# zbqq/neus2

Hardware: AMD Instinct MI355X
Metric: training samples/sec (compacted NeuS2 training samples, DTU-scan24-shaped synthetic, base.json) (higher is better)
Workload: dtype fp16 MFMA (fp32 accumulate) / fp32 optimizer; 1 GPU; NeuS2 train step, Config S, base.json L=14 T=2^19 W=64, Nc=2^18/GPU, R=2^18/GPU fixed, all 14 levels active (network trained 800 steps before the warm-up); global_batch=262144, rays_per_gpu=262144, parallelism=dp1, prepare_steps=800, levels_active=14

## Files before the change

include/neus2_hip.h:

```cpp
#ifndef NEUS2_HIP_H
#define NEUS2_HIP_H

#include <stdint.h>

#ifdef __cplusplus
extern "C" {
#endif

typedef struct NeusTestbed NeusTestbed;

typedef struct NeusNetworkConfig {
	uint32_t n_levels;
	uint32_t n_features_per_level;
	uint32_t log2_hashmap_size;
	uint32_t base_resolution;
	float per_level_scale;
	float top_resolution;
	float valid_level_scale;
	float base_valid_level_scale;
	uint32_t base_training_step;
	uint32_t n_neurons;
	uint32_t n_density_hidden;
	uint32_t n_rgb_hidden;
	float learning_rate, beta1, beta2, epsilon, l2_reg;
// ... 154 lines not shown
int neus_testbed_ray_counts(NeusTestbed* tb, uint32_t n, uint32_t* nreq, uint32_t* ccount, uint32_t* numsteps );
int neus_debug_time_kernel(NeusTestbed* tb, int kernel, int variant, int iters, float* ms_out);
int neus_testbed_time_kernel(NeusTestbed* tb, int kernel, int iters, float* ms_out, uint32_t* units_out);
int neus_debug_march_stats(NeusTestbed* tb, uint32_t n, uint32_t* out);
int neus_debug_march_profile(NeusTestbed* tb, unsigned long long* out, uint32_t max_waves, uint32_t* n_waves);
int neus_debug_scatter_stats(NeusTestbed* tb, uint64_t* records_per_level, uint32_t* max_region);
int neus_debug_scatter_parts(NeusTestbed* tb, uint32_t* parts_per_level );
int neus_debug_grid_scatter(NeusTestbed* tb, void* hip_stream, uint32_t n_cap, const uint32_t* n_valid, const float* coords,
                            uint32_t coord_stride, uint32_t valid_level, const void* dLdenc, const void* genc, const float* v,
                            float* grid_grad_out);
int neus_debug_mlp_train(NeusTestbed* tb, void* hip_stream, uint32_t n, const float* coords, const uint16_t* enc, const float* dydx,
                         const uint16_t* dL_dout, uint32_t indeed_batch_size, float* grads_out, float* dpos, uint16_t* genc_out,
                         uint16_t* dLdenc_out, uint16_t* d1_delta_out, float* v_out);
int neus_debug_exclusive_scan(void* hip_stream, const uint32_t* in, uint32_t* out, uint32_t n, int reps, uint32_t* failures);
int neus_debug_scan_giveup(void* hip_stream, const uint32_t* in, uint32_t* out, uint32_t n, uint32_t* failures);
int neus_debug_inject_health(NeusTestbed* tb, uint32_t flags);
int neus_debug_set_lds_fill(NeusTestbed* tb, uint32_t pattern);
int neus_debug_set_lds_fill_all(NeusTestbed* tb, uint32_t pattern);
int neus_debug_set_xcd_shift(NeusTestbed* tb, uint32_t n_blocks);
int neus_debug_set_grid_generic(uint32_t on);
int neus_debug_get_batch(NeusTestbed* tb, float* coords_out, uint16_t* dl_dout_out, float* loss_out);
int neus_debug_denorm_probe(int device, uint32_t n, uint32_t launches, uint64_t* stats);
int neus_debug_get_buffer(NeusTestbed* tb, int id, uint64_t offset, uint64_t nbytes, void* host);
int neus_debug_replay_loss_grad(NeusTestbed* tb, uint16_t* dl_dout_out);
int neus_debug_sample_rays_round0(NeusTestbed* tb, void* stream, uint32_t n_rays, uint32_t n_rays_total, uint64_t rng_state, uint64_t rng_inc,
                                  uint32_t max_samples, const uint8_t* bitfield, float* rays, uint32_t* numsteps, float* coords,
                                  uint32_t* counters_out, uint32_t chunk_end, uint32_t* list, uint32_t* list_len, uint32_t lds_fill);
int neus_testbed_stream(NeusTestbed* tb, void** hip_stream);
int neus_testbed_synchronize(NeusTestbed* tb);
#define NEUS_N_PHASES 10
// ... 110 lines not shown
```

neus2_amd/_lib.py:

```python
from __future__ import annotations

import ctypes as C
import os

_HERE = os.path.dirname(os.path.abspath(__file__))
LIB_PATH = os.environ.get("NEUS2_HIP_LIB") or os.path.join(_HERE, "libneus2_hip.so")


class NeusNetworkConfig(C.Structure):
    _fields_ = [
        ("n_levels", C.c_uint32), ("n_features_per_level", C.c_uint32), ("log2_hashmap_size", C.c_uint32),
        ("base_resolution", C.c_uint32), ("per_level_scale", C.c_float), ("top_resolution", C.c_float),
        ("valid_level_scale", C.c_float), ("base_valid_level_scale", C.c_float), ("base_training_step", C.c_uint32),
        ("n_neurons", C.c_uint32), ("n_density_hidden", C.c_uint32), ("n_rgb_hidden", C.c_uint32),
        ("learning_rate", C.c_float), ("beta1", C.c_float), ("beta2", C.c_float), ("epsilon", C.c_float), ("l2_reg", C.c_float),
        ("ema_decay", C.c_float), ("decay_start", C.c_uint32), ("decay_interval", C.c_uint32), ("decay_base", C.c_float),
        ("ek_loss_weight", C.c_float), ("mask_loss_weight", C.c_float), ("anneal_end", C.c_uint32), ("batch_size", C.c_uint32),
        ("sdf_bias", C.c_float), ("density_grid_decay", C.c_float), ("seed", C.c_uint32), ("fixed_rays_per_batch", C.c_uint32),
        ("predict_global_movement", C.c_uint32), ("global_movement_steps", C.c_uint32), ("finetune_global_movement", C.c_uint32),
        ("reset_density_grid_after_global_movement", C.c_uint32), ("after_learning_rate", C.c_float),
        ("gm_learning_rate", C.c_float), ("gm_beta1", C.c_float), ("gm_beta2", C.c_float), ("gm_epsilon", C.c_float),
        ("gm_decay_start", C.c_uint32), ("gm_decay_interval", C.c_uint32), ("gm_decay_base", C.c_float),
    ]

# ... 68 lines not shown

class NeusModuleInfo(C.Structure):
    _fields_ = [("n_params", C.c_uint64), ("n_input_dims", C.c_uint32), ("n_output_dims", C.c_uint32),
                ("param_precision", C.c_int32), ("output_precision", C.c_int32), ("gradient_precision", C.c_int32),
                ("batch_capacity", C.c_uint32), ("n_levels", C.c_uint32), ("grid_offset", C.c_uint64),
                ("per_level_scale", C.c_float)]


EXPORTS = [
    "neus_last_error", "neus_abi_version", "neus_device_count", "neus_device_synchronize",
    "neus_testbed_create", "neus_testbed_destroy", "neus_testbed_set_dataset", "neus_testbed_reload_network",
    "neus_testbed_layout", "neus_testbed_train", "neus_testbed_get_stats", "neus_testbed_get_params",
    "neus_testbed_set_params", "neus_testbed_get_gradients", "neus_testbed_get_ema_params",
    "neus_testbed_get_half_params",
    "neus_testbed_get_density_grid", "neus_testbed_set_density_grid", "neus_testbed_restore_state", "neus_testbed_get_rng", "neus_testbed_render", "neus_testbed_sdf_on_grid",
    "neus_testbed_marching_cubes", "neus_testbed_mc_density", "neus_testbed_get_mesh", "neus_testbed_mesh_vertex_colors", "neus_mc_table", "neus_prepare_image_rgba8", "neus_testbed_ray_counts", "neus_debug_time_kernel", "neus_debug_march_stats", "neus_debug_exclusive_scan", "neus_debug_scan_giveup", "neus_debug_inject_health", "neus_debug_set_lds_fill", "neus_debug_set_lds_fill_all", "neus_debug_set_xcd_shift", "neus_debug_set_grid_generic", "neus_debug_denorm_probe", "neus_debug_get_batch", "neus_debug_get_buffer", "neus_debug_replay_loss_grad", "neus_debug_sample_rays_round0", "neus_debug_march_profile", "neus_debug_scatter_stats", "neus_debug_scatter_parts", "neus_debug_grid_scatter", "neus_debug_mlp_train", "neus_testbed_time_kernel", "neus_testbed_stream",
    "neus_testbed_synchronize", "neus_testbed_set_profiling", "neus_testbed_kernel_times", "neus_testbed_set_infer_timing", "neus_testbed_infer_timing",
    "neus_testbed_set_exchange_timing", "neus_testbed_exchange_timing",
    "neus_nccl_unique_id", "neus_testbed_init_data_parallel", "neus_testbed_init_data_parallel_ex",
    "neus_testbed_data_parallel_info", "neus_testbed_set_exchange_overlap", "neus_local_group_create", "neus_local_group_destroy",
    "neus_testbed_init_local_group", "neus_host_group_create", "neus_host_group_destroy", "neus_testbed_init_host_group", "neus_debug_host_group_allreduce",
    "neus_grid_encode", "neus_net_forward", "neus_net_backward", "neus_sample_rays", "neus_loss_compact",
    "neus_optimizer_step", "neus_fill_rollover", "neus_occ_update", "neus_mfma_probe",
    "neus_testbed_next_frame", "neus_testbed_get_movement", "neus_testbed_set_movement", "neus_testbed_frame_state",
    "neus_testbed_change_frame", "neus_testbed_prepare_for_test", "neus_testbed_get_training_options",
    "neus_testbed_set_training_options", "neus_testbed_saved_transform", "neus_testbed_get_optimizer_state",
    "neus_testbed_set_optimizer_state", "neus_testbed_set_progressive_inference",
    "neus_module_create_network", "neus_module_create_nerf_network", "neus_module_create_encoding", "neus_module_create_network_with_input_encoding", "neus_module_destroy", "neus_context_destroy",
    "neus_module_info", "neus_module_hyperparams", "neus_module_set_training_step", "neus_module_set_indeed_batch_size",
    "neus_module_initialize_params", "neus_module_inference", "neus_module_forward", "neus_module_backward",
    "neus_module_backward_backward_input",
# ... 39 lines not shown
```

neus2_amd/csrc/kernels.h:

```cpp
#pragma once
#include <functional>
#include <vector>
#include "common.h"

namespace neus {

struct MlpPtrs {
	const half_t* d0;  const half_t* d1;
	const half_t* r0;  const half_t* r1;  const half_t* r2;
	const half_t* d0T; const half_t* d1T;
	const half_t* r0T; const half_t* r1T; const half_t* r2T;
	const half_t* d0p; const half_t* d0Tp;
	const half_t* var;
	float sdf_bias;
};

struct TrainBufs {
	half_t* d1_delta;
	half_t* dLdenc; half_t* genc;
	float4* v;
	float* var_grad;
	float* var_partial;
	float indeed_batch;
	float4* dpos;
// ... 87 lines not shown

struct LossWork {
	float4* sa;
	float4* ck4;
	float* cke;
	float* ekt;
	uint32_t* sample_ray;
	const uint32_t* rbase;
	float4* racc;
	float* rT;
	float* rek;
	uint32_t* long_rays;
	uint32_t* n_long;
	float4* rgr;
	uint32_t* cmap;
};

constexpr uint32_t ADAM_BIAS_TAB = 4096;
struct AdamParams {
	uint32_t n, n_matrix;
	float loss_scale, lr, beta1, beta2, eps, l2_reg;
	float ema_decay, ema_debias_old, ema_debias_new;
	uint32_t optimize_matrix, optimize_non_matrix;
	const float* bias_tab;
	uint32_t bias_converged;
	float inv_loss_scale;
	uint32_t pow2_scale;
	uint32_t skip_ema_h;
	const uint32_t* abort;
};
// ... 278 lines not shown
```

neus2_amd/csrc/march.hip:

```cpp
#pragma clang fp contract(off)
#include "march_common.h"
#include "scan_lookback.h"
#include <algorithm>
#include <cstdlib>
#include <cstring>
#include <vector>

namespace neus {



__global__ void k_bitfield_linear(const uint8_t* __restrict__ bf, uint32_t* __restrict__ lin) {
	const uint32_t w = blockIdx.x * blockDim.x + threadIdx.x;
	if (w >= GRID3 / 32) return;
	const uint32_t ix = w >> 9, iy = (w >> 2) & 127, iz0 = (w & 3) * 32;
	uint32_t word = 0;
	for (uint32_t b = 0; b < 32; ++b) {
		const uint32_t idx = morton3D(ix, iy, iz0 + b);
		word |= (uint32_t)((bf[idx / 8] >> (idx % 8)) & 1) << b;
	}
	lin[w] = word;
}
__device__ __forceinline__ bool ray_hits_box(const float o[3], const float d[3], const float bb[6]) {
	float tn = 0.0f, tf = 3.402823466e+38f;
// ... 1143 lines not shown
						for (uint32_t j = lane; j < m_o; j += 64) list[p_o + j] = s_o + j;
					}
				}
				if (rays_out) {
					const unsigned long long mk = __ballot(m > 0);
					uint32_t q0 = 0;
					if (lane == 0) q0 = atomicAdd(n_rays_out, (uint32_t)__popcll(mk));
					q0 = wave_lane_value(q0, 0);
					if (m > 0) rays_out[q0 + (uint32_t)__popcll(mk & ((1ull << lane) - 1ull))] = i;
				}
			}
		}
	}
}

__global__ void __launch_bounds__(256) k_prog_cut(uint32_t cap_rays, const uint32_t* __restrict__ ccount, const uint32_t* __restrict__ excl,
                                                  uint32_t batch, uint32_t* __restrict__ cutw, int mode, uint32_t* __restrict__ eval0,
                                                  uint32_t* __restrict__ abort_if_none) {
	const uint32_t i = blockIdx.x * blockDim.x + threadIdx.x;
	if (i >= cap_rays) return;
	const uint32_t e = excl[i], incl = e + ccount[i];
	const bool cross = e < batch && incl >= batch, none = i == cap_rays - 1 && incl < batch;
	if (!cross && !none) return;
	const uint32_t c = cross ? i : cap_rays;
	if (mode == 0) {
		cutw[CW_CUT_A] = c;
		cutw[CW_LENB_EFF] = cross ? 0u : cutw[CW_LENB];
		cutw[CW_NB_EFF] = cross ? 0u : cutw[CW_NB];
	} else {
		cutw[CW_CUT] = c;
// ... 92 lines not shown
                                                  float4* __restrict__ racc, const float* __restrict__ rT, float4* __restrict__ rgr,
                                                  float* __restrict__ loss_out, float* __restrict__ ek_out, float* __restrict__ mask_out,
                                                  uint32_t* __restrict__ cmap) {
	const uint32_t lane = threadIdx.x & 63;
	const uint32_t R = st->rays_per_batch;
	const uint32_t n_rays_global = R * dp.world, n_rays_total = st->n_rays_total;
	const uint32_t cap64 = (cap_rays + 63u) & ~63u;
	const uint32_t mi_lb = st->mi_lb;
	if (lp.abort_w && blockIdx.x == 0 && threadIdx.x == 0) lp.abort_w[lp.abort_slot ^ 1u] = 0u;
	for (uint32_t i = blockIdx.x * blockDim.x + threadIdx.x; i < cap64; i += gridDim.x * blockDim.x) {
		uint32_t comp = 0, cb = 0;
		if (i < cap_rays) {
			const uint32_t ns = numsteps[2 * i], base = numsteps[2 * i + 1];
			const uint32_t cn = ccount[i];
			cb = cbase[i];
			if (i == cap_rays - 1) {
				if (lp.abort_w && st->march_cut && cb + cn < lp.max_compacted) lp.abort_w[lp.abort_slot] = 1u;
				st->compacted_counter = cb + cn;
				st->compacted_global = cb + cn;
				st->rays_ws_global = st->n_rays_with_samples;
				st->n_train = min(cb + cn, lp.max_compacted) ? lp.max_compacted : 0u;
			}
			loss_out[i] = 0.f; ek_out[i] = 0.f; mask_out[i] = 0.f;
			if (ns == 0) {
				numsteps[2 * i] = 0; numsteps[2 * i + 1] = cb;
			} else {
				const float4 acc = racc[i];
				float rgb_ray[3] = {acc.x, acc.y, acc.z}, weight_sum = acc.w;
				const float T = rT[i];
				const uint32_t ig = dp.rank * R + i;
				pcg32 rng(lp.rng_state, lp.rng_inc);
				pcg_advance(rng, (uint64_t)(uint32_t)(ig * N_MAX_RANDOM_SAMPLES_PER_RAY), lp.jt);
				const uint32_t img = image_idx(ig, n_rays_global, n_rays_total, ds.n_images);
				const int rx = ds.res[2 * img], ry = ds.res[2 * img + 1];
				float xx, yy; random_image_pos(rng, rx, ry, xx, yy);
				float bg[3];
				if (ds.target.fixed_bg) { bg[0] = ds.target.bg[0]; bg[1] = ds.target.bg[1]; bg[2] = ds.target.bg[2]; }
				else { bg[0] = rng.next_float(); bg[1] = rng.next_float(); bg[2] = rng.next_float(); }
	#pragma unroll
				for (int k = 0; k < 3; ++k) bg[k] = srgb_to_linear(bg[k]);
				float tex[4]; read_rgba(ds, img, xx, yy, tex);
				float target[3];
				const uint32_t tmode = ds.target.mode;
	#pragma unroll
				for (int k = 0; k < 3; ++k) {
					if (tmode != 1) {
						target[k] = 1.0f * tex[k] + (1.0f - tex[3]) * bg[k];
						if (tmode == 0) { target[k] = linear_to_srgb(target[k]); bg[k] = linear_to_srgb(bg[k]); }
					} else {
						bg[k] = linear_to_srgb(bg[k]);
						target[k] = tex[3] > 0.0f ? linear_to_srgb(1.0f * tex[k] / tex[3]) * tex[3] + (1.0f - tex[3]) * bg[k] : bg[k];
					}
				}
				if (cn == ns) {
	#pragma unroll
					for (int k = 0; k < 3; ++k) rgb_ray[k] += T * bg[k];
				}
				comp = min(lp.max_compacted - min(lp.max_compacted, cb), cn);
				if (lp.abort_w && mi_lb && comp > 0 && base + ns > mi_lb) lp.abort_w[lp.abort_slot] = 1u;
				numsteps[2 * i] = comp; numsteps[2 * i + 1] = cb;
				if (comp > 0) {
					float lgrad[3], lloss[3];
	#pragma unroll
					for (int k = 0; k < 3; ++k) {
						const float diff = rgb_ray[k] - target[k], ad = fabsf(diff), sq = 0.5f / 0.1f * diff * diff;
						lloss[k] = (ad > 0.1f ? (ad - 0.5f * 0.1f) : sq) / 5.0f;
						lgrad[k] = (ad > 0.1f ? (diff > 0 ? 1.0f : -1.0f) : (diff / 0.1f)) / 5.0f;
					}
					const float mask_gt = (float)(tex[3] > 0.9999f);
					float gws;
					if (weight_sum >= 1.0 - 1e-4) { weight_sum = 1.0 - 1e-4; gws = 0.0f; }
					else if (weight_sum <= 1e-4) { weight_sum = 1e-4; gws = 0.0f; }
					else { const float sws = 1.0f / (1.0f + exp(-(double)weight_sum)); gws = (mask_gt - sws) * weight_sum * lp.mask_w; }
					const float mean_loss = ((lloss[0] + lloss[1]) + lloss[2]) / 3.0f;
					loss_out[i] = mean_loss / (float)n_rays_global;
					mask_out[i] = -(mask_gt * logf(weight_sum) + (1 - mask_gt) * logf(1 - weight_sum));
					float Tb;
					const RecState sc = scan_replay(base, base + comp - 1, sa, ekt, ck4, cke, Tb);
					ek_out[i] = sc.ek / ((float)comp * (float)n_rays_global);
					rgr[i] = make_float4(lgrad[0], lgrad[1], lgrad[2], gws * (1 - weight_sum));
					racc[i] = make_float4(rgb_ray[0], rgb_ray[1], rgb_ray[2], 0.f);
				}
			}
		}
		unsigned long long todo = __ballot(comp > 0);
		const uint32_t i0 = i - lane;
		while (todo) {
			const int o = __ffsll(todo) - 1;
			todo &= todo - 1ull;
			const uint32_t c_o = wave_lane_value(comp, o), d_o = wave_lane_value(cb, o);
			for (uint32_t j = lane; j < c_o; j += 64) cmap[d_o + j] = i0 + (uint32_t)o;
		}
	}
}
// ... 244 lines not shown
void launch_loss_alpha(hipStream_t s, uint32_t cap_samples, const StepState* st, const float* coords, const half_t* net_out, float cos_anneal,
                       const LossWork& w, bool dt_const) {
	dbg_lds_gate(s);
	k_loss_alpha<<<sample_blocks(cap_samples), 256, 0, s>>>(cap_samples, &st->n_kept, nullptr, coords, net_out, cos_anneal, w.sa, w.ekt, w.n_long,
	                                                        dt_const);
}
void launch_loss_alpha_list(hipStream_t s, uint32_t cap_samples, const uint32_t* n_ptr, const uint32_t* idx, const float* coords,
                            const half_t* net_out, float cos_anneal, const LossWork& w, bool dt_const) {
	dbg_lds_gate(s);
	k_loss_alpha<<<sample_blocks(cap_samples), 256, 0, s>>>(cap_samples, n_ptr, idx, coords, net_out, cos_anneal, w.sa, w.ekt, nullptr, dt_const);
}
void launch_loss_scan_chunk(hipStream_t s, uint32_t cap_rays, const uint32_t* numsteps, const LossWork& w, uint32_t* ccount, uint32_t e0,
                            uint32_t e1, uint32_t e2, uint32_t* list, uint32_t* next_counter, const uint32_t* rays_in, const uint32_t* n_rays_in,
                            uint32_t* rays_out, uint32_t* n_rays_out) {
	dbg_lds_gate(s);
	k_loss_scan_chunk<<<std::max<uint32_t>(1, std::min<uint32_t>((cap_rays + 63) / 64, 8192)), 64, 0, s>>>(
		cap_rays, numsteps, w.sa, w.ekt, w.ck4, w.cke, ccount, w.racc, w.rT, w.rek, e0, e1, e2, list, next_counter, rays_in, n_rays_in,
		rays_out, n_rays_out);
}
void launch_prog_cut(hipStream_t s, uint32_t cap_rays, const uint32_t* ccount, const uint32_t* excl, uint32_t batch, uint32_t* cutw, int mode,
                     uint32_t* eval0, uint32_t* abort_if_none) {
	k_prog_cut<<<(cap_rays + 255) / 256, 256, 0, s>>>(cap_rays, ccount, excl, batch, cutw, mode, eval0, abort_if_none);
}
void launch_prog_next(hipStream_t s, uint32_t cap_rays, const uint32_t* rays_in, const uint32_t* n_in, const uint32_t* numsteps, const uint32_t* cut,
                      uint32_t e1, uint32_t e2, uint32_t* list, uint32_t* list_counter, uint32_t* rays_out, uint32_t* n_out) {
	k_prog_next<<<std::max<uint32_t>(1, std::min<uint32_t>((cap_rays + 255) / 256, 1024)), 256, 0, s>>>(rays_in, n_in, numsteps, cut, e1, e2, list,
	                                                                                                   list_counter, rays_out, n_out);
}
void launch_loss_scan_ray(hipStream_t s, uint32_t cap_rays, const uint32_t* numsteps, const LossWork& w, uint32_t* ccount) {
	const uint32_t blocks = ray_blocks(cap_rays);
	dbg_lds_gate(s);
	k_loss_scan_ray<true><<<blocks, 256, 0, s>>>(cap_rays, numsteps, w.sa, w.ekt, w.ck4, w.cke, ccount, w.racc, w.rT, w.long_rays, w.n_long);
	if (w.long_rays) dbg_lds_gate(s);
// ... 44 lines not shown
```

neus2_amd/csrc/march_common.h:

```cpp
#pragma once
#pragma clang fp contract(off)
#include "kernels.h"

namespace neus {

__device__ __forceinline__ float clampf(float v, float lo, float hi) { return v < lo ? lo : (v > hi ? hi : v); }
__device__ __forceinline__ float calc_dt(float t, float cone) { return clampf(t * cone, MIN_CONE_STEPSIZE, MAX_CONE_STEPSIZE); }
__device__ __forceinline__ float warp_dt(float dt) {
	const float max_stepsize = MIN_CONE_STEPSIZE * (1 << (NERF_CASCADES - 1));
	return (dt - MIN_CONE_STEPSIZE) / (max_stepsize - MIN_CONE_STEPSIZE);
}
__device__ __forceinline__ float unwarp_dt(float dt) {
	const float max_stepsize = MIN_CONE_STEPSIZE * (1 << (NERF_CASCADES - 1));
	return dt * (max_stepsize - MIN_CONE_STEPSIZE) + MIN_CONE_STEPSIZE;
}
__device__ __forceinline__ int clampi(int v, int lo, int hi) { return v < lo ? lo : (v > hi ? hi : v); }
__device__ __forceinline__ uint32_t cascaded_grid_idx_at(float px, float py, float pz, uint32_t mip) {
	const float s = scalbnf(1.0f, -(int)mip);
	px = ((px - 0.5f) * s) + 0.5f; py = ((py - 0.5f) * s) + 0.5f; pz = ((pz - 0.5f) * s) + 0.5f;
	const int ix = (int)(px * NERF_GRIDSIZE), iy = (int)(py * NERF_GRIDSIZE), iz = (int)(pz * NERF_GRIDSIZE);
	return morton3D(clampi(ix, 0, NERF_GRIDSIZE - 1), clampi(iy, 0, NERF_GRIDSIZE - 1), clampi(iz, 0, NERF_GRIDSIZE - 1));
}
__device__ __forceinline__ bool occupied(float px, float py, float pz, const uint8_t* bf, uint32_t mip) {
	const uint32_t idx = cascaded_grid_idx_at(px, py, pz, mip);
// ... 41 lines not shown
	do { t += calc_dt(t, cone); } while (t < t_target);
	return t;
}
__device__ __forceinline__ float srgb_to_linear(float s) { return s <= 0.04045f ? s / 12.92f : powf((s + 0.055f) / 1.055f, 2.4f); }
__device__ __forceinline__ float linear_to_srgb(float l) { return l < 0.0031308f ? 12.92f * l : 1.055f * powf(l, 0.41666f) - 0.055f; }

__device__ __forceinline__ uint32_t image_idx(uint32_t base_idx, uint32_t n_rays, uint32_t n_rays_total, uint32_t n_img) {
	return (((base_idx + n_rays_total) * n_img) / n_rays) % n_img;
}
__device__ __forceinline__ void random_image_pos(pcg32& rng, int rx, int ry, float& x, float& y) {
	x = rng.next_float(); y = rng.next_float();
	const int ix = min(max((int)(x * (float)rx), 0), rx - 1);
	const int iy = min(max((int)(y * (float)ry), 0), ry - 1);
	x = ((float)ix + 0.5f) / (float)rx; y = ((float)iy + 0.5f) / (float)ry;
}
__device__ __forceinline__ void read_rgba(const DevDataset& ds, uint32_t img, float x, float y, float o[4]) {
	const int rx = ds.res[2 * img], ry = ds.res[2 * img + 1];
	const int px = clampi((int)(x * (float)rx), 0, rx - 1), py = clampi((int)(y * (float)ry), 0, ry - 1);
	const uint32_t v = ds.pixels[ds.pix_off[img] + (uint64_t)px + (uint64_t)py * rx];
	if (v == 0x00FF00FFu) { o[0] = o[1] = o[2] = o[3] = -1.0f; return; }
	const float a = (float)((v >> 24) & 0xff) * (1.0f / 255.0f);
	o[0] = ds.lin_lut[v & 0xff] * a;
	o[1] = ds.lin_lut[(v >> 8) & 0xff] * a;
	o[2] = ds.lin_lut[(v >> 16) & 0xff] * a;
	o[3] = a;
}
__device__ __forceinline__ bool aabb_contains(const DevDataset& ds, const float p[3]) {
	return (p[0] >= ds.aabb_min[0]) & (p[0] <= ds.aabb_max[0]) & (p[1] >= ds.aabb_min[1]) & (p[1] <= ds.aabb_max[1]) &
	       (p[2] >= ds.aabb_min[2]) & (p[2] <= ds.aabb_max[2]);
}
__device__ __forceinline__ void ray_intersect(const DevDataset& ds, const float o[3], const float d[3], float& tmin_o) {
	float tmin = (ds.aabb_min[0] - o[0]) / d[0], tmax = (ds.aabb_max[0] - o[0]) / d[0];
	if (tmin > tmax) { float t = tmin; tmin = tmax; tmax = t; }
	float tymin = (ds.aabb_min[1] - o[1]) / d[1], tymax = (ds.aabb_max[1] - o[1]) / d[1];
	if (tymin > tymax) { float t = tymin; tymin = tymax; tymax = t; }
	const float FM = 3.402823466e+38f;
	if (tmin > tymax || tymin > tmax) { tmin_o = FM; return; }
	if (tymin > tmin) tmin = tymin;
	if (tymax < tmax) tmax = tymax;
	float tzmin = (ds.aabb_min[2] - o[2]) / d[2], tzmax = (ds.aabb_max[2] - o[2]) / d[2];
// ... 99 lines not shown
```

neus2_amd/csrc/options.h:

```cpp
#pragma once

#include <algorithm>
#include <cstdint>
#include <cstdio>
#include <cstdlib>
#include <cstring>
#include <vector>

namespace neus_env {
inline bool on_unless_0(const char* name) { const char* e = std::getenv(name); return !(e && e[0] == '0'); }
inline bool off_unless_1(const char* name) { const char* e = std::getenv(name); return e && e[0] == '1'; }
inline bool is(const char* name, const char* value) { const char* e = std::getenv(name); return e && std::strcmp(e, value) == 0; }
inline int as_int(const char* name, int def) { const char* e = std::getenv(name); return e ? std::atoi(e) : def; }
inline uint32_t as_u32(const char* name, uint32_t def) { const char* e = std::getenv(name); return e ? (uint32_t)std::strtoul(e, nullptr, 10) : def; }
inline float as_float(const char* name, float def) { const char* e = std::getenv(name); return e ? (float)std::atof(e) : def; }
inline std::vector<uint32_t> increasing_list(const char* name) {
	std::vector<uint32_t> v;
	const char* e = std::getenv(name);
	if (!e) return v;
	for (const char* p = e; *p;) { char* q = nullptr; const unsigned long x = std::strtoul(p, &q, 10); if (q == p) break; v.push_back((uint32_t)x); p = *q ? q + 1 : q; }
	bool ok = !v.empty() && v.size() <= 14 && v[0] > 0;
	for (size_t k = 1; k < v.size(); ++k) ok = ok && v[k] > v[k - 1];
	if (!ok) v.clear();
	return v;
// ... 13 lines not shown
	bool eager_ema_h = false;

	uint32_t march_waves = 0;
	uint32_t march_lanes = 8;
	bool march_balance = true;
	uint32_t march_dbg = 0;
	bool ray_cull = true;
	bool ray_sort = true;
	bool prog_cut = true;
	bool march_cut = true;
	uint32_t march_cut_div = 1;
	std::vector<uint32_t> chunk_ends;
	float chunk_scale = 2.f;
	int chunk_rounds = 2;

	bool occ_sort = true;
	bool occ_nu_sort = false;

	uint32_t scatter_mode = 2;
	uint32_t scatter_chunk = 512;
	uint32_t scatter_level_groups = 0;
	uint32_t scatter_xcd_group = 4;
	bool scatter_noskip = false;

	bool dbg_loss_replay = false;
	bool dbg_loss_fence = false;

	static NeusOptions from_env() {
		using namespace neus_env;
		NeusOptions o;
// ... 7 lines not shown
		o.adam_overlap = off_unless_1("NEUS_ADAM_OVERLAP");
		o.exchange_overlap = on_unless_0("NEUS_EXCHANGE_OVERLAP");
		o.eager_ema_h = off_unless_1("NEUS_EAGER_EMA_H");
		o.march_waves = as_u32("NEUS_MARCH_WAVES", o.march_waves);
		{ const uint32_t v = as_u32("NEUS_MARCH_LANES", 8); o.march_lanes = v == 1 || v == 4 || v == 16 ? v : 8u; }
		o.march_balance = on_unless_0("NEUS_MARCH_BALANCE");
		o.march_dbg = as_u32("NEUS_MARCH_DBG", o.march_dbg);
		o.ray_cull = on_unless_0("NEUS_RAY_CULL");
		o.ray_sort = on_unless_0("NEUS_RAY_SORT");
		o.prog_cut = on_unless_0("NEUS_PROG_CUT");
		o.march_cut = on_unless_0("NEUS_MARCH_CUT");
		o.march_cut_div = (uint32_t)std::max(1, as_int("NEUS_DBG_MARCH_CUT_DIV", 1));
		o.chunk_ends = increasing_list("NEUS_CHUNK_ENDS");
		o.chunk_scale = as_float("NEUS_CHUNK_SCALE", o.chunk_scale);
		o.chunk_rounds = as_int("NEUS_CHUNK_ROUNDS", o.chunk_rounds);
		o.occ_sort = on_unless_0("NEUS_OCC_SORT");
		o.occ_nu_sort = off_unless_1("NEUS_OCC_NU_SORT");
		o.scatter_mode = is("NEUS_SCATTER", "binned") ? 1u : is("NEUS_SCATTER", "wide") ? 0u : 2u;
		o.scatter_chunk = is("NEUS_SCATTER_CHUNK", "1024") ? 1024u : is("NEUS_SCATTER_CHUNK", "256") ? 256u : 512u;
		if (o.scatter_mode != 2 && o.scatter_chunk == 256) o.scatter_chunk = 512;
		o.scatter_level_groups = (uint32_t)std::max(0, as_int("NEUS_SCATTER_LG", 0));
		o.scatter_xcd_group = std::max(1u, as_u32("NEUS_SC_XCD_GROUP", o.scatter_xcd_group));
		o.scatter_noskip = off_unless_1("NEUS_SCATTER_NOSKIP");
		o.dbg_loss_replay = off_unless_1("NEUS_DBG_LOSS_REPLAY");
		o.dbg_loss_fence = off_unless_1("NEUS_DBG_LOSS_FENCE");
		return o;
	}
};

struct NeusProcessOptions {
// ... 32 lines not shown
```

neus2_amd/csrc/testbed.cpp:

```cpp
#include <rocprofiler-sdk-roctx/roctx.h>
#include "kernels.h"
#include "scan_lookback.h"
#include "json_lite.h"
#include "hostgroup.h"
#include "options.h"
#include "../../include/neus2_hip.h"

#include <rccl/rccl.h>

#include <algorithm>
#include <atomic>
#include <cstdio>
#include <functional>
#include <chrono>
#include <cmath>
#include <condition_variable>
#include <mutex>
#include <cstdlib>
#include <cstring>
#include <memory>
#include <random>
#include <stdexcept>
#include <string>
#include <vector>
// ... 1696 lines not shown
		launch_march_count(s, MAX_RAYS, max_samples, st.p, dp, ds, bitfield.p, bf_lin.p, r.state, r.inc, rays.p, startt.p, nreq.p, mw,
		                   progressive ? chunk_cnt.p : nullptr, RAW_CNT + nch, opt.ray_cull ? occ_bbox.p : nullptr);
		launch_march_write(s, MAX_RAYS, st.p, ds, rays.p, mw, nreq.p, base.p, numsteps.p, coords.p, nullptr, max_samples, scan,
		                   progressive && !sorted_rays ? &r0 : nullptr, dbg_lds_fill);
		const RaySort rsort{rs_hist.p, rs_off.p, rs_key.p, rs_perm.p, chunk_cnt.p + RS_N_PERM};
		const RaySplit split{cutw.p + CW_EST, ccount.p, cutw.p, MAX_RAYS, max_samples};
		if (sorted_rays)
			launch_ray_sort(s, MAX_RAYS, numsteps.p, coords.p, ce[0], rsort, chunk_list.p, chunk_cnt.p, scan, scan_tmp_bytes, cut ? &split : nullptr);
	}

	LossWork loss_work(const uint32_t* rbase) {
		LossWork w{};
		w.sa = l_sa.p; w.ck4 = l_ck4.p; w.cke = l_cke.p; w.ekt = l_ekt.p; w.sample_ray = sample_ray.p; w.rbase = rbase; w.cmap = cmap.p;
		w.racc = l_racc.p; w.rT = l_rT.p; w.rgr = l_rgr.p; w.rek = l_rek.p;
		w.long_rays = long_rays.p; w.n_long = chunk_cnt.p + 16;
		return w;
	}

	void accumulate_phases(int par) {
		HIP_CHECK(hipEventSynchronize(ev_done[par]));
		for (int i = 0; i < N_PHASES; ++i) {
			float ms = 0.f;
			HIP_CHECK(hipEventElapsedTime(&ms, ev[par][i], ev[par][i + 1]));
			phase_ms[i] += ms;
		}
		const StepState& h = prof_st[par];
		phase_npre += h.n_kept;
		phase_ntrain += std::min(h.compacted_global / std::max(1u, world), batch);
		++phase_steps;
		prof_pending[par] = false;
// ... 923 lines not shown
	return guard([&] {
		if (chunk_end == 0 || !list || !list_len) throw std::runtime_error("sample_rays_round0: chunk_end > 0, list and list_len required");
		sample_rays_impl(tb, stream, n_rays, 0u, 1u, n_rays_total, rng_state, rng_inc, max_samples, bitfield, rays, numsteps, coords, counters_out,
		                 chunk_end, list, list_len, lds_fill);
	});
}
int neus_debug_scan_giveup(void* stream, const uint32_t* in, uint32_t* out, uint32_t n, uint32_t* failures) {
	return guard([&] {
		hipStream_t s = (hipStream_t)stream;
		ScanTemp tmp; tmp.alloc(scan_temp_bytes(n) + 256); scan_temp_reset(s, tmp.p);
		debug_scan_skip_first_tile(s, tmp.p, in, out, n);
		HIP_CHECK(hipStreamSynchronize(s));
		*failures = scan_failures(tmp.p);
	});
}
int neus_debug_set_lds_fill(NeusTestbed* tb, uint32_t pattern) { return guard([&] { tb->dbg_lds_fill = pattern; }); }
int neus_debug_set_lds_fill_all(NeusTestbed* tb, uint32_t pattern) { return guard([&] { tb->dbg_lds_fill_all = pattern; }); }
int neus_debug_set_xcd_shift(NeusTestbed* tb, uint32_t n_blocks) { return guard([&] { tb->dbg_xcd_shift = n_blocks; }); }
int neus_debug_set_grid_generic(uint32_t on) { return guard([&] { g_dbg_grid_generic = on; }); }
int neus_debug_denorm_probe(int device, uint32_t n, uint32_t launches, uint64_t* stats) {
	return guard([&] {
		if (!stats || n == 0) throw std::runtime_error("neus_debug_denorm_probe: bad argument");
		HIP_CHECK(hipSetDevice(device));
		hipStream_t s = nullptr;
		HIP_CHECK(hipStreamCreateWithFlags(&s, hipStreamNonBlocking));
		try { debug_denorm_probe(s, n, launches, stats); } catch (...) { (void)hipStreamDestroy(s); throw; }
		HIP_CHECK(hipStreamDestroy(s));
	});
}
int neus_debug_get_buffer(NeusTestbed* tb, int id, uint64_t offset, uint64_t nbytes, void* host) {
// ... 1370 lines not shown
```

Before: 342.9 million samples/s.

## Add warp-specialized chunked loss scan and replace final replay with checkpoint lookup

Adds a new loss-scan kernel in which two loader waves stage per-ray sample tiles into double-buffered LDS while a recurrence wave runs the transmittance scan and writes checkpoints. This hides global-memory latency behind the serial per-ray recurrence. It is used by default for every round except the first one that builds a list. The finalize kernel now rebuilds the eikonal sum from the nearest checkpoint plus at most SCAN_CK samples instead of a full scan_replay. It also hoists the pixel, LUT and accumulator loads earlier so their latency overlaps other work. The cost is more threads and LDS per block, plus added complexity and a new debug entry point.

```diff
diff --git a/include/neus2_hip.h b/include/neus2_hip.h
--- a/include/neus2_hip.h
+++ b/include/neus2_hip.h
@@ -192,6 +192,10 @@
                          uint16_t* dLdenc_out, uint16_t* d1_delta_out, float* v_out);
 int neus_debug_exclusive_scan(void* hip_stream, const uint32_t* in, uint32_t* out, uint32_t n, int reps, uint32_t* failures);
 int neus_debug_scan_giveup(void* hip_stream, const uint32_t* in, uint32_t* out, uint32_t n, uint32_t* failures);
+int neus_debug_loss_scan_rounds(void* hip_stream, uint32_t n_rays, uint32_t n_samples, const uint32_t* numsteps, const float* sa,
+                                const float* ekt, const uint32_t* perm, uint32_t n_perm, const uint32_t* ends, uint32_t n_ends, int legacy,
+                                uint32_t* ccount, float* racc, float* rT, float* rek, float* ck4, float* cke, uint32_t* lists,
+                                uint32_t* list_len, uint32_t* open_rays, uint32_t* n_open);
 int neus_debug_inject_health(NeusTestbed* tb, uint32_t flags);
 int neus_debug_set_lds_fill(NeusTestbed* tb, uint32_t pattern);
 int neus_debug_set_lds_fill_all(NeusTestbed* tb, uint32_t pattern);
diff --git a/neus2_amd/_lib.py b/neus2_amd/_lib.py
--- a/neus2_amd/_lib.py
+++ b/neus2_amd/_lib.py
@@ -106,7 +106,7 @@
     "neus_testbed_set_params", "neus_testbed_get_gradients", "neus_testbed_get_ema_params",
     "neus_testbed_get_half_params",
     "neus_testbed_get_density_grid", "neus_testbed_set_density_grid", "neus_testbed_restore_state", "neus_testbed_get_rng", "neus_testbed_render", "neus_testbed_sdf_on_grid",
-    "neus_testbed_marching_cubes", "neus_testbed_mc_density", "neus_testbed_get_mesh", "neus_testbed_mesh_vertex_colors", "neus_mc_table", "neus_prepare_image_rgba8", "neus_testbed_ray_counts", "neus_debug_time_kernel", "neus_debug_march_stats", "neus_debug_exclusive_scan", "neus_debug_scan_giveup", "neus_debug_inject_health", "neus_debug_set_lds_fill", "neus_debug_set_lds_fill_all", "neus_debug_set_xcd_shift", "neus_debug_set_grid_generic", "neus_debug_denorm_probe", "neus_debug_get_batch", "neus_debug_get_buffer", "neus_debug_replay_loss_grad", "neus_debug_sample_rays_round0", "neus_debug_march_profile", "neus_debug_scatter_stats", "neus_debug_scatter_parts", "neus_debug_grid_scatter", "neus_debug_mlp_train", "neus_testbed_time_kernel", "neus_testbed_stream",
+    "neus_testbed_marching_cubes", "neus_testbed_mc_density", "neus_testbed_get_mesh", "neus_testbed_mesh_vertex_colors", "neus_mc_table", "neus_prepare_image_rgba8", "neus_testbed_ray_counts", "neus_debug_time_kernel", "neus_debug_march_stats", "neus_debug_exclusive_scan", "neus_debug_scan_giveup", "neus_debug_loss_scan_rounds", "neus_debug_inject_health", "neus_debug_set_lds_fill", "neus_debug_set_lds_fill_all", "neus_debug_set_xcd_shift", "neus_debug_set_grid_generic", "neus_debug_denorm_probe", "neus_debug_get_batch", "neus_debug_get_buffer", "neus_debug_replay_loss_grad", "neus_debug_sample_rays_round0", "neus_debug_march_profile", "neus_debug_scatter_stats", "neus_debug_scatter_parts", "neus_debug_grid_scatter", "neus_debug_mlp_train", "neus_testbed_time_kernel", "neus_testbed_stream",
     "neus_testbed_synchronize", "neus_testbed_set_profiling", "neus_testbed_kernel_times", "neus_testbed_set_infer_timing", "neus_testbed_infer_timing",
     "neus_testbed_set_exchange_timing", "neus_testbed_exchange_timing",
     "neus_nccl_unique_id", "neus_testbed_init_data_parallel", "neus_testbed_init_data_parallel_ex",
diff --git a/neus2_amd/csrc/kernels.h b/neus2_amd/csrc/kernels.h
--- a/neus2_amd/csrc/kernels.h
+++ b/neus2_amd/csrc/kernels.h
@@ -125,6 +125,7 @@
 	uint32_t* n_long;
 	float4* rgr;
 	uint32_t* cmap;
+	uint32_t scan_impl;
 };
 
 constexpr uint32_t ADAM_BIAS_TAB = 4096;
diff --git a/neus2_amd/csrc/march.hip b/neus2_amd/csrc/march.hip
--- a/neus2_amd/csrc/march.hip
+++ b/neus2_amd/csrc/march.hip
@@ -1181,6 +1181,186 @@
 	}
 }
 
+constexpr uint32_t SW_TILE = 16, SW_PAD = SW_TILE + 1, SW_LOADERS = 2, SW_THREADS = 64 * (SW_LOADERS + 1);
+static_assert(SW_TILE == 2 * SCAN_CK, "a tile holds two checkpoints per ray (slots 0 and 1; slot 2 is the sink)");
+typedef float sw_f4v __attribute__((ext_vector_type(4)));
+template <uint32_t u>
+__device__ __forceinline__ void sw_steps(RayScan& S, uint32_t& p, uint32_t cnt, uint32_t k0, const sw_f4v (&x)[SW_TILE], const float (&y)[SW_TILE],
+                                         sw_f4v* c4, float* ce) {
+	if constexpr (u < SW_TILE) {
+		if (u >= cnt || S.T < 1e-4f) return;
+		const uint32_t slot = (u & (SCAN_CK - 1)) == k0 ? u / SCAN_CK : 2u;
+		c4[slot * 64] = sw_f4v{S.T, S.r0, S.r1, S.r2}; ce[slot * 64] = S.ek;
+		const float w = x[u][0] * S.T;
+		S.r0 = S.r0 + w * x[u][1]; S.r1 = S.r1 + w * x[u][2]; S.r2 = S.r2 + w * x[u][3];
+		S.ws = S.ws + w; S.ek = S.ek + y[u]; S.T = S.T * (1.f - x[u][0]);
+		++p;
+		sw_steps<u + 1>(S, p, cnt, k0, x, y, c4, ce);
+	}
+}
+__global__ void __launch_bounds__(SW_THREADS) k_loss_scan_chunk_wg(uint32_t cap_rays, const uint32_t* __restrict__ numsteps, const float4* __restrict__ sa,
+                                                                   const float* __restrict__ ekt, float4* __restrict__ ck4, float* __restrict__ cke,
+                                                                   uint32_t* __restrict__ ccount, float4* __restrict__ racc, float* __restrict__ rT,
+                                                                   float* __restrict__ rek, uint32_t e0, uint32_t e1, uint32_t e2,
+                                                                   uint32_t* __restrict__ list, uint32_t* __restrict__ next_counter,
+                                                                   const uint32_t* __restrict__ rays_in, const uint32_t* __restrict__ n_rays_in,
+                                                                   uint32_t* __restrict__ rays_out, uint32_t* __restrict__ n_rays_out) {
+	constexpr uint32_t U = SW_TILE, PAD = SW_PAD, RPL = 64 / SW_LOADERS, RPI = 64 / U, NJ = RPL / RPI;
+	typedef sw_f4v f4v;
+	__shared__ f4v s_q[2][64 * PAD];
+	__shared__ float s_e[2][64 * PAD];
+	__shared__ f4v s_c4[2][3 * 64];
+	__shared__ float s_ce[2][3 * 64];
+	__shared__ uint32_t s_p[2][64];
+	__shared__ uint32_t s_g0[64], s_gl[64], s_m[64], s_pre[64], s_src[64];
+	__shared__ uint32_t s_nt, s_go[2], s_tot, s_p0;
+	const uint32_t wid = threadIdx.x >> 6, lane = threadIdx.x & 63;
+	const bool rec = wid == 0;
+	const uint32_t ld = wid - 1, sub = lane / U, el = lane % U;
+	const char* sab = (const char*)sa;
+	const char* ekb = (const char*)ekt;
+	const uint32_t n_slots = rays_in ? min(*n_rays_in, cap_rays) : cap_rays;
+	for (uint32_t w0 = blockIdx.x * 64; w0 < n_slots; w0 += gridDim.x * 64) {
+		uint32_t i = 0, ns = 0, base = 0, nsamp = 0, k0 = 0;
+		RayScan S{1.f, 0.f, 0.f, 0.f, 0.f, 0.f, 0u};
+		bool open = false, live = false;
+		if (rec) {
+			const bool inr = w0 + lane < n_slots;
+			i = rays_in ? (inr ? rays_in[w0 + lane] : 0u) : w0 + lane;
+			ns = inr ? numsteps[2 * i] : 0u; base = inr ? numsteps[2 * i + 1] : 0u;
+			open = inr && (e0 == 0 || ns > 0);
+			if (e0 > 0 && inr) {
+				const uint32_t cn = ccount[i];
+				const float T = rT[i];
+				const float4 a = racc[i];
+				const float ek = rek[i];
+				S.cn = cn;
+				if (!open || cn != e0 || e0 >= ns || T < 1e-4f) open = false;
+				else { S.T = T; S.r0 = a.x; S.r1 = a.y; S.r2 = a.z; S.ws = a.w; S.ek = ek; }
+			}
+			const uint32_t to = min(ns, e1);
+			live = open && to > e0;
+			nsamp = live ? to - e0 : 0u;
+			const uint32_t g0 = live ? base + e0 : 0u;
+			s_g0[lane] = g0; s_gl[lane] = live ? g0 + nsamp - 1u : 0u;
+			k0 = (SCAN_CK - (g0 & (SCAN_CK - 1))) & (SCAN_CK - 1);
+			uint32_t nmax = nsamp;
+#pragma unroll
+			for (int d = 32; d; d >>= 1) nmax = max(nmax, (uint32_t)__shfl_xor((int)nmax, d));
+			if (lane == 0) s_nt = (nmax + U - 1) / U;
+		}
+		__syncthreads();
+		const uint32_t nt = s_nt;
+		if (nt) {
+			uint32_t lb[NJ], ll[NJ];
+			f4v qa[NJ], qb[NJ]; float ea[NJ], eb[NJ];
+			auto fetch = [&](f4v (&q)[NJ], float (&e)[NJ], uint32_t t) {
+#pragma unroll
+				for (uint32_t j = 0; j < NJ; ++j) {
+					const uint32_t g = min(lb[j] + t * U + el, ll[j]);
+					q[j] = *(const f4v*)(sab + ((size_t)g << 4));
+					e[j] = *(const float*)(ekb + ((size_t)g << 2));
+				}
+			};
+			auto stage = [&](const f4v (&q)[NJ], const float (&e)[NJ], uint32_t par) {
+#pragma unroll
+				for (uint32_t j = 0; j < NJ; ++j) {
+					const uint32_t r = RPL * ld + RPI * j + sub;
+					s_q[par][r * PAD + el] = q[j]; s_e[par][r * PAD + el] = e[j];
+				}
+			};
+			auto drain = [&](uint32_t t, uint32_t par) {
+				if (lane < 2 * RPL) {
+					const uint32_t r = RPL * ld + (lane >> 1), h = lane & 1u;
+					const uint32_t g0 = s_g0[r], pos = ((SCAN_CK - (g0 & (SCAN_CK - 1))) & (SCAN_CK - 1)) + SCAN_CK * h;
+					if (pos < s_p[par][r]) {
+						const uint32_t en = (g0 + t * U + pos) / SCAN_CK;
+						const f4v c = s_c4[par][h * 64 + r];
+						ck4[en] = make_float4(c[0], c[1], c[2], c[3]); cke[en] = s_ce[par][h * 64 + r];
+					}
+				}
+			};
+			if (!rec) {
+#pragma unroll
+				for (uint32_t j = 0; j < NJ; ++j) { const uint32_t r = RPL * ld + RPI * j + sub; lb[j] = s_g0[r]; ll[j] = s_gl[r]; }
+				fetch(qa, ea, 0); fetch(qb, eb, 1);
+				stage(qa, ea, 0);
+				fetch(qa, ea, 2);
+			}
+			__syncthreads();
+			auto tile = [&](uint32_t t, f4v (&q)[NJ], float (&e)[NJ], const uint32_t par) -> bool {
+				if (rec) {
+					uint32_t p = 0;
+					if (live) {
+						const uint32_t c = t * U, cnt = min(nsamp - c, U);
+						f4v x[U]; float y[U];
+#pragma unroll
+						for (uint32_t u = 0; u < U; ++u) { x[u] = s_q[par][lane * PAD + u]; y[u] = s_e[par][lane * PAD + u]; }
+#pragma unroll
+						for (uint32_t u = 0; u < U; ++u) asm volatile("" : "+v"(x[u]), "+v"(y[u]));
+						sw_steps<0>(S, p, cnt, k0, x, y, &s_c4[par][lane], &s_ce[par][lane]);
+						S.cn += p;
+						live = p == U && c + U < nsamp && !(S.T < 1e-4f);
+					}
+					s_p[par][lane] = p;
+					const bool any = __ballot(live) != 0;
+					if (lane == 0) s_go[par] = any ? 1u : 0u;
+				} else {
+					stage(q, e, par ^ 1u);
+					fetch(q, e, t + 3);
+					if (t > 0) drain(t - 1, par ^ 1u);
+				}
+				__syncthreads();
+				return s_go[par] != 0;
+			};
+			uint32_t t = 0;
+			for (;;) {
+				if (!tile(t, qb, eb, 0u) || t + 1 >= nt) break;
+				++t;
+				if (!tile(t, qa, ea, 1u) || t + 1 >= nt) break;
+				++t;
+			}
+			if (!rec) drain(t, t & 1u);
+		}
+		if (rec && open) {
+			ccount[i] = S.cn;
+			racc[i] = make_float4(S.r0, S.r1, S.r2, S.ws);
+			rT[i] = S.T;
+			rek[i] = S.ek;
+		}
+		if (list || rays_out) {
+			if (rec) {
+				const uint32_t m = (open && S.cn == e1 && e1 < ns && S.T >= 1e-4f) ? min(ns, e2) - e1 : 0u;
+				const uint32_t incl = wave_incl_sum(m);
+				const uint32_t total = wave_lane_value(incl, 63);
+				const unsigned long long mk = __ballot(m > 0);
+				uint32_t p0 = 0, q0 = 0;
+				if (lane == 0 && total) {
+					if (list) p0 = atomicAdd(next_counter, total);
+					if (rays_out) q0 = atomicAdd(n_rays_out, (uint32_t)__popcll(mk));
+				}
+				if (list) {
+					s_m[lane] = m; s_pre[lane] = incl - m; s_src[lane] = base + e1;
+					if (lane == 0) { s_tot = total; s_p0 = p0; }
+				}
+				q0 = wave_lane_value(q0, 0);
+				if (rays_out && m > 0) rays_out[q0 + (uint32_t)__popcll(mk & ((1ull << lane) - 1ull))] = i;
+			}
+			if (list) {
+				__syncthreads();
+				if (s_tot) {
+					const uint32_t p0 = s_p0;
+					for (uint32_t o = wid; o < 64; o += SW_LOADERS + 1) {
+						const uint32_t m_o = s_m[o], p_o = p0 + s_pre[o], s_o = s_src[o];
+						for (uint32_t j = lane; j < m_o; j += 64) list[p_o + j] = s_o + j;
+					}
+				}
+			}
+		}
+		__syncthreads();
+	}
+}
+
 __global__ void __launch_bounds__(256) k_prog_cut(uint32_t cap_rays, const uint32_t* __restrict__ ccount, const uint32_t* __restrict__ excl,
                                                   uint32_t batch, uint32_t* __restrict__ cutw, int mode, uint32_t* __restrict__ eval0,
                                                   uint32_t* __restrict__ abort_if_none) {
@@ -1303,6 +1483,8 @@
 			const uint32_t ns = numsteps[2 * i], base = numsteps[2 * i + 1];
 			const uint32_t cn = ccount[i];
 			cb = cbase[i];
+			const float4 acc = racc[i];
+			const float T = rT[i];
 			if (i == cap_rays - 1) {
 				if (lp.abort_w && st->march_cut && cb + cn < lp.max_compacted) lp.abort_w[lp.abort_slot] = 1u;
 				st->compacted_counter = cb + cn;
@@ -1314,21 +1496,33 @@
 			if (ns == 0) {
 				numsteps[2 * i] = 0; numsteps[2 * i + 1] = cb;
 			} else {
-				const float4 acc = racc[i];
 				float rgb_ray[3] = {acc.x, acc.y, acc.z}, weight_sum = acc.w;
-				const float T = rT[i];
+				comp = min(lp.max_compacted - min(lp.max_compacted, cb), cn);
+				const uint32_t s_last = base + (comp ? comp - 1u : 0u), g_ck = s_last & ~(SCAN_CK - 1);
+				const bool from_ck = g_ck > base;
+				const uint32_t k_first = from_ck ? g_ck : base, n_rep = comp ? s_last - k_first + 1u : 0u;
+				const float ck_e = cke[(from_ck ? g_ck : base) / SCAN_CK];
+				float e_rep[SCAN_CK];
+	#pragma unroll
+				for (uint32_t j = 0; j < SCAN_CK; ++j) e_rep[j] = ekt[min(k_first + j, s_last)];
 				const uint32_t ig = dp.rank * R + i;
+				const uint32_t img = image_idx(ig, n_rays_global, n_rays_total, ds.n_images);
+				const int rx = ds.res[2 * img], ry = ds.res[2 * img + 1];
+				const uint64_t pix0 = ds.pix_off[img];
+				asm volatile("" ::: "memory");
 				pcg32 rng(lp.rng_state, lp.rng_inc);
 				pcg_advance(rng, (uint64_t)(uint32_t)(ig * N_MAX_RANDOM_SAMPLES_PER_RAY), lp.jt);
-				const uint32_t img = image_idx(ig, n_rays_global, n_rays_total, ds.n_images);
-				const int rx = ds.res[2 * img], ry = ds.res[2 * img + 1];
 				float xx, yy; random_image_pos(rng, rx, ry, xx, yy);
+				const uint32_t pix = read_pixel(ds, rx, ry, pix0, xx, yy);
+				asm volatile("" ::: "memory");
 				float bg[3];
 				if (ds.target.fixed_bg) { bg[0] = ds.target.bg[0]; bg[1] = ds.target.bg[1]; bg[2] = ds.target.bg[2]; }
 				else { bg[0] = rng.next_float(); bg[1] = rng.next_float(); bg[2] = rng.next_float(); }
-	#pragma unroll
-				for (int k = 0; k < 3; ++k) bg[k] = srgb_to_linear(bg[k]);
-				float tex[4]; read_rgba(ds, img, xx, yy, tex);
+				bg[0] = srgb_to_linear(bg[0]);
+				float lut[3]; pixel_lut(ds, pix, lut);
+				asm volatile("" ::: "memory");
+				bg[1] = srgb_to_linear(bg[1]); bg[2] = srgb_to_linear(bg[2]);
+				float tex[4]; decode_rgba(pix, lut, tex);
 				float target[3];
 				const uint32_t tmode = ds.target.mode;
 	#pragma unroll
@@ -1345,7 +1539,6 @@
 	#pragma unroll
 					for (int k = 0; k < 3; ++k) rgb_ray[k] += T * bg[k];
 				}
-				comp = min(lp.max_compacted - min(lp.max_compacted, cb), cn);
 				if (lp.abort_w && mi_lb && comp > 0 && base + ns > mi_lb) lp.abort_w[lp.abort_slot] = 1u;
 				numsteps[2 * i] = comp; numsteps[2 * i + 1] = cb;
 				if (comp > 0) {
@@ -1364,9 +1557,10 @@
 					const float mean_loss = ((lloss[0] + lloss[1]) + lloss[2]) / 3.0f;
 					loss_out[i] = mean_loss / (float)n_rays_global;
 					mask_out[i] = -(mask_gt * logf(weight_sum) + (1 - mask_gt) * logf(1 - weight_sum));
-					float Tb;
-					const RecState sc = scan_replay(base, base + comp - 1, sa, ekt, ck4, cke, Tb);
-					ek_out[i] = sc.ek / ((float)comp * (float)n_rays_global);
+					float ek_sum = from_ck ? ck_e : 0.f;
+	#pragma unroll
+					for (uint32_t j = 0; j < SCAN_CK; ++j) ek_sum = j < n_rep ? ek_sum + e_rep[j] : ek_sum;
+					ek_out[i] = ek_sum / ((float)comp * (float)n_rays_global);
 					rgr[i] = make_float4(lgrad[0], lgrad[1], lgrad[2], gws * (1 - weight_sum));
 					racc[i] = make_float4(rgb_ray[0], rgb_ray[1], rgb_ray[2], 0.f);
 				}
@@ -1641,9 +1835,14 @@
                             uint32_t e1, uint32_t e2, uint32_t* list, uint32_t* next_counter, const uint32_t* rays_in, const uint32_t* n_rays_in,
                             uint32_t* rays_out, uint32_t* n_rays_out) {
 	dbg_lds_gate(s);
-	k_loss_scan_chunk<<<std::max<uint32_t>(1, std::min<uint32_t>((cap_rays + 63) / 64, 8192)), 64, 0, s>>>(
-		cap_rays, numsteps, w.sa, w.ekt, w.ck4, w.cke, ccount, w.racc, w.rT, w.rek, e0, e1, e2, list, next_counter, rays_in, n_rays_in,
-		rays_out, n_rays_out);
+	const uint32_t blocks = std::max<uint32_t>(1, std::min<uint32_t>((cap_rays + 63) / 64, 8192));
+	const bool legacy = w.scan_impl == 1 || (w.scan_impl == 0 && e0 == 0 && list);
+	if (legacy)
+		k_loss_scan_chunk<<<blocks, 64, 0, s>>>(cap_rays, numsteps, w.sa, w.ekt, w.ck4, w.cke, ccount, w.racc, w.rT, w.rek, e0, e1, e2, list,
+		                                        next_counter, rays_in, n_rays_in, rays_out, n_rays_out);
+	else
+		k_loss_scan_chunk_wg<<<blocks, SW_THREADS, 0, s>>>(cap_rays, numsteps, w.sa, w.ekt, w.ck4, w.cke, ccount, w.racc, w.rT, w.rek, e0, e1, e2,
+		                                                   list, next_counter, rays_in, n_rays_in, rays_out, n_rays_out);
 }
 void launch_prog_cut(hipStream_t s, uint32_t cap_rays, const uint32_t* ccount, const uint32_t* excl, uint32_t batch, uint32_t* cutw, int mode,
                      uint32_t* eval0, uint32_t* abort_if_none) {
diff --git a/neus2_amd/csrc/march_common.h b/neus2_amd/csrc/march_common.h
--- a/neus2_amd/csrc/march_common.h
+++ b/neus2_amd/csrc/march_common.h
@@ -79,16 +79,25 @@
 	const int iy = min(max((int)(y * (float)ry), 0), ry - 1);
 	x = ((float)ix + 0.5f) / (float)rx; y = ((float)iy + 0.5f) / (float)ry;
 }
-__device__ __forceinline__ void read_rgba(const DevDataset& ds, uint32_t img, float x, float y, float o[4]) {
-	const int rx = ds.res[2 * img], ry = ds.res[2 * img + 1];
+__device__ __forceinline__ uint32_t read_pixel(const DevDataset& ds, int rx, int ry, uint64_t pix_off, float x, float y) {
 	const int px = clampi((int)(x * (float)rx), 0, rx - 1), py = clampi((int)(y * (float)ry), 0, ry - 1);
-	const uint32_t v = ds.pixels[ds.pix_off[img] + (uint64_t)px + (uint64_t)py * rx];
+	return ds.pixels[pix_off + (uint64_t)px + (uint64_t)py * rx];
+}
+__device__ __forceinline__ void pixel_lut(const DevDataset& ds, uint32_t v, float lut[3]) {
+	lut[0] = ds.lin_lut[v & 0xff]; lut[1] = ds.lin_lut[(v >> 8) & 0xff]; lut[2] = ds.lin_lut[(v >> 16) & 0xff];
+}
+__device__ __forceinline__ void decode_rgba(uint32_t v, const float lut[3], float o[4]) {
 	if (v == 0x00FF00FFu) { o[0] = o[1] = o[2] = o[3] = -1.0f; return; }
 	const float a = (float)((v >> 24) & 0xff) * (1.0f / 255.0f);
-	o[0] = ds.lin_lut[v & 0xff] * a;
-	o[1] = ds.lin_lut[(v >> 8) & 0xff] * a;
-	o[2] = ds.lin_lut[(v >> 16) & 0xff] * a;
+	o[0] = lut[0] * a;
+	o[1] = lut[1] * a;
+	o[2] = lut[2] * a;
 	o[3] = a;
+}
+__device__ __forceinline__ void read_rgba(const DevDataset& ds, uint32_t img, float x, float y, float o[4]) {
+	const uint32_t v = read_pixel(ds, ds.res[2 * img], ds.res[2 * img + 1], ds.pix_off[img], x, y);
+	float lut[3]; pixel_lut(ds, v, lut);
+	decode_rgba(v, lut, o);
 }
 __device__ __forceinline__ bool aabb_contains(const DevDataset& ds, const float p[3]) {
 	return (p[0] >= ds.aabb_min[0]) & (p[0] <= ds.aabb_max[0]) & (p[1] >= ds.aabb_min[1]) & (p[1] <= ds.aabb_max[1]) &
diff --git a/neus2_amd/csrc/options.h b/neus2_amd/csrc/options.h
--- a/neus2_amd/csrc/options.h
+++ b/neus2_amd/csrc/options.h
@@ -51,6 +51,8 @@
 	float chunk_scale = 2.f;
 	int chunk_rounds = 2;
 
+	uint32_t scan_impl = 0;
+
 	bool occ_sort = true;
 	bool occ_nu_sort = false;
 
@@ -88,6 +90,7 @@
 		o.chunk_ends = increasing_list("NEUS_CHUNK_ENDS");
 		o.chunk_scale = as_float("NEUS_CHUNK_SCALE", o.chunk_scale);
 		o.chunk_rounds = as_int("NEUS_CHUNK_ROUNDS", o.chunk_rounds);
+		o.scan_impl = is("NEUS_SCAN_IMPL", "legacy") ? 1u : is("NEUS_SCAN_IMPL", "wg") ? 2u : 0u;
 		o.occ_sort = on_unless_0("NEUS_OCC_SORT");
 		o.occ_nu_sort = off_unless_1("NEUS_OCC_NU_SORT");
 		o.scatter_mode = is("NEUS_SCATTER", "binned") ? 1u : is("NEUS_SCATTER", "wide") ? 0u : 2u;
diff --git a/neus2_amd/csrc/testbed.cpp b/neus2_amd/csrc/testbed.cpp
--- a/neus2_amd/csrc/testbed.cpp
+++ b/neus2_amd/csrc/testbed.cpp
@@ -1734,6 +1734,7 @@
 		w.sa = l_sa.p; w.ck4 = l_ck4.p; w.cke = l_cke.p; w.ekt = l_ekt.p; w.sample_ray = sample_ray.p; w.rbase = rbase; w.cmap = cmap.p;
 		w.racc = l_racc.p; w.rT = l_rT.p; w.rgr = l_rgr.p; w.rek = l_rek.p;
 		w.long_rays = long_rays.p; w.n_long = chunk_cnt.p + 16;
+		w.scan_impl = opt.scan_impl;
 		return w;
 	}
 
@@ -2687,6 +2688,39 @@
 		*failures = scan_failures(tmp.p);
 	});
 }
+int neus_debug_loss_scan_rounds(void* stream, uint32_t n_rays, uint32_t n_samples, const uint32_t* numsteps, const float* sa, const float* ekt,
+                                const uint32_t* perm, uint32_t n_perm, const uint32_t* ends, uint32_t n_ends, int legacy, uint32_t* ccount,
+                                float* racc, float* rT, float* rek, float* ck4, float* cke, uint32_t* lists, uint32_t* list_len,
+                                uint32_t* open_rays, uint32_t* n_open) {
+	return guard([&] {
+		if (n_rays == 0 || n_samples == 0 || n_ends > 14 || (n_ends && !ends) || (perm && n_perm > n_rays))
+			throw std::runtime_error("neus_debug_loss_scan_rounds: bad argument");
+		if (!numsteps || !sa || !ekt || !ccount || !racc || !rT || !rek || !ck4 || !cke || (n_ends && (!lists || !list_len || !open_rays || !n_open)))
+			throw std::runtime_error("neus_debug_loss_scan_rounds: null buffer");
+		for (uint32_t k = 0; k < n_ends; ++k)
+			if (ends[k] == 0 || (k && ends[k] <= ends[k - 1])) throw std::runtime_error("neus_debug_loss_scan_rounds: ends must be positive and increasing");
+		hipStream_t s = (hipStream_t)stream;
+		Dev<uint32_t> np; np.alloc(1);
+		HIP_CHECK(hipMemcpyAsync(np.p, &n_perm, 4, hipMemcpyHostToDevice, s));
+		if (n_ends) {
+			HIP_CHECK(hipMemsetAsync(list_len, 0, 4 * (size_t)n_ends, s));
+			HIP_CHECK(hipMemsetAsync(n_open, 0, 4 * (size_t)n_ends, s));
+		}
+		LossWork w{};
+		w.sa = (float4*)sa; w.ekt = (float*)ekt; w.ck4 = (float4*)ck4; w.cke = cke; w.racc = (float4*)racc; w.rT = rT; w.rek = rek;
+		w.scan_impl = legacy ? 1u : 2u;
+		uint32_t e0 = 0;
+		for (uint32_t k = 0; k <= n_ends; ++k) {
+			const uint32_t e1 = k < n_ends ? ends[k] : 0xffffffffu, e2 = k + 1 < n_ends ? ends[k + 1] : 0xffffffffu;
+			const bool more = k < n_ends;
+			launch_loss_scan_chunk(s, n_rays, numsteps, w, ccount, e0, e1, e2, more ? lists + (size_t)k * n_samples : nullptr,
+			                       more ? list_len + k : nullptr, k ? open_rays + (size_t)(k - 1) * n_rays : perm, k ? n_open + (k - 1) : (perm ? np.p : nullptr),
+			                       more ? open_rays + (size_t)k * n_rays : nullptr, more ? n_open + k : nullptr);
+			e0 = e1;
+		}
+		HIP_CHECK(hipStreamSynchronize(s));
+	});
+}
 int neus_debug_set_lds_fill(NeusTestbed* tb, uint32_t pattern) { return guard([&] { tb->dbg_lds_fill = pattern; }); }
 int neus_debug_set_lds_fill_all(NeusTestbed* tb, uint32_t pattern) { return guard([&] { tb->dbg_lds_fill_all = pattern; }); }
 int neus_debug_set_xcd_shift(NeusTestbed* tb, uint32_t n_blocks) { return guard([&] { tb->dbg_xcd_shift = n_blocks; }); }
```

Result: no change. 345.2 million samples/s (median of 6 runs) (+0.7%).
